# adityamwagh/SuperSLAM

Hardware: AMD Instinct MI355X
Metric: stereo pairs/sec (SPx2+LG) at 1376x376 (higher is better)
Workload: dtype f16; 1 GPU; configs[1]: SuperPoint x2 + select + gather + 1x LightGlue on 1376x376 stereo pairs; a step = 8 x 64 = 512 pairs per GPU resident in HBM (8 library calls of 64 pairs, different images per call), max_keypoints 600, seeded synthetic weights; pairs_per_call=64, max_keypoints=600, matches_last_call=1412, parallelism=replicated weights, pairs sharded over 1 rank(s), no data-path collective

## Files before the change

superslam_amd/csrc/sp_convs.hip:

```cpp
#include <cstdlib>
#include <string>

#include "igemm.h"
#include "kernels.h"

namespace sship {

static IgemmArgs conv_args(const ConvW& w, const _Float16* in, int B, int H, int W) {
  IgemmArgs a{};
  a.in0 = in; a.in1 = in; a.cin0 = w.cin; a.cs0 = w.cin; a.cs1 = w.cin;
  a.wpack = w.w; a.bias = w.bias; a.B = B; a.H = H; a.W = W; a.cout = w.cout; a.ostride = w.cout;
  return a;
}

hipError_t sp_conv1x1_f16(const ConvW& w, const _Float16* in, _Float16* out, int B, int H, int W, hipStream_t s) {
  IgemmArgs a = conv_args(w, in, B, H, W);
  a.out0 = out;
  if (w.cin != 256) return hipErrorInvalidValue;
  return launch_igemm<1, 256, 128, 4, EpiF16<false, false>>(a, w.cout_pad, s);
}

typedef float f4x_t __attribute__((ext_vector_type(4)));
__global__ __launch_bounds__(256, 2) void k_convpb_stream(const _Float16* __restrict__ in, const _Float16* __restrict__ w,
                                                          const float* __restrict__ bias, float* __restrict__ out, int P,
                                                          int ostride) {
  __shared__ __attribute__((aligned(16))) _Float16 s_a4[8 * 512];
  const int lane = threadIdx.x & 63, n = lane & 15, kb = lane >> 4;
  for (int u = threadIdx.x; u < 8 * 64; u += 256) {
    const int ks = u >> 6, l = u & 63;
    *reinterpret_cast<uint4*>(s_a4 + u * 8) = *reinterpret_cast<const uint4*>(w + (size_t)(64 + (l & 15)) * 256 + ks * 32 + (l >> 4) * 8);
  }
  h8_t a[4][8];
#pragma unroll
  for (int m = 0; m < 4; ++m)
#pragma unroll
    for (int ks = 0; ks < 8; ++ks) a[m][ks] = *reinterpret_cast<const h8_t*>(w + (size_t)(16 * m + n) * 256 + ks * 32 + kb * 8);
  __shared__ __attribute__((aligned(16))) float s_b[80];
  if (threadIdx.x < 80) s_b[threadIdx.x] = threadIdx.x < 65 ? bias[threadIdx.x] : 0.f;
  __syncthreads();
  const int ntiles = (P + 15) >> 4, nwaves = gridDim.x * 4;
  const _Float16* src = in + kb * 8;
  h8_t fA[8], fB[8];
  auto fetch = [&](h8_t (&f)[8], int t) __attribute__((always_inline)) {
    const int pix = min(min(t, ntiles - 1) * 16 + n, P - 1);
    const _Float16* p = src + (size_t)pix * 256;
#pragma unroll
    for (int ks = 0; ks < 8; ++ks) f[ks] = *reinterpret_cast<const h8_t*>(p + ks * 32);
  };
  auto tile = [&](const h8_t (&f)[8], int t) __attribute__((always_inline)) {
    f4x_t acc[5];
#pragma unroll
    for (int m = 0; m < 5; ++m) acc[m] = *reinterpret_cast<const f4x_t*>(s_b + 16 * m + 4 * kb);
#pragma unroll
    for (int ks = 0; ks < 8; ++ks) {
      const h8_t a4 = *reinterpret_cast<const h8_t*>(s_a4 + (ks * 64 + lane) * 8);
#pragma unroll
      for (int m = 0; m < 4; ++m) acc[m] = __builtin_amdgcn_mfma_f32_16x16x32_f16(a[m][ks], f[ks], acc[m], 0, 0, 0);
      acc[4] = __builtin_amdgcn_mfma_f32_16x16x32_f16(a4, f[ks], acc[4], 0, 0, 0);
    }
    const int pix = t * 16 + n;
    if (pix < P) {
      float* o = out + (size_t)pix * ostride + 4 * kb;
#pragma unroll
      for (int m = 0; m < 4; ++m) *reinterpret_cast<f4x_t*>(o + 16 * m) = acc[m];
      if (kb == 0) o[64] = acc[4][0];
    }
  };
  const int t0 = blockIdx.x * 4 + (threadIdx.x >> 6);
  fetch(fA, t0);
  for (int t = t0; t < ntiles; t += 2 * nwaves) {
    fetch(fB, t + nwaves);
    __builtin_amdgcn_sched_barrier(0);
    tile(fA, t);
    if (t + nwaves < ntiles) {
      fetch(fA, t + 2 * nwaves);
      __builtin_amdgcn_sched_barrier(0);
      tile(fB, t + nwaves);
    }
  }
}

hipError_t sp_conv1x1_f32(const ConvW& w, const _Float16* in, float* out, int ostride, int B, int H, int W,
                          hipStream_t s) {
  if (w.cin != 256) return hipErrorInvalidValue;
  static const bool use_igemm = dev_env("SUPERSLAM_HIP_CONVPB") && std::string(dev_env("SUPERSLAM_HIP_CONVPB")) == "igemm";
  if (w.w_q && w.cout == 65 && ostride >= 68 && ostride % 4 == 0 && !use_igemm) {
    const int P = B * H * W;
    int wgs = 2 * cu_count();
    if (wgs * 4 > (P + 15) / 16) wgs = ((P + 15) / 16 + 3) / 4;
    hipLaunchKernelGGL(k_convpb_stream, dim3(wgs), dim3(256), 0, s, in, w.w_q, w.bias, out, P, ostride);
    return hipGetLastError();
  }
#if SSHIP_DEV_SWITCHES
  IgemmArgs a = conv_args(w, in, B, H, W);
  a.out0 = out; a.ostride = ostride;
  return launch_igemm<1, 256, 96, 4, EpiF32>(a, w.cout_pad, s);
#else
  return hipErrorInvalidValue;
#endif
}

constexpr int kDhLd = 264;
__global__ __launch_bounds__(512) void k_desc_head_gather(const _Float16* __restrict__ da, int Hc, int Wc,
                                                          const int* __restrict__ cell_h, const int* __restrict__ cell_w,
                                                          const int* __restrict__ n_dev, int max_kp,
                                                          const _Float16* __restrict__ wp, const float* __restrict__ bias,
                                                          _Float16* __restrict__ out, size_t out_img_stride) {
  __shared__ __attribute__((aligned(16))) _Float16 s_x[64 * kDhLd];
  __shared__ float s_red[8][64];
  const int b = blockIdx.y, i0 = blockIdx.x * 64;
  const int n = n_dev[b];
  if (i0 >= n) return;
  const int tid = threadIdx.x, wave = tid >> 6, lane = tid & 63, j = lane & 31, hh = lane >> 5;
  const _Float16* img = da + (size_t)b * Hc * Wc * 256;
  for (int u = tid; u < 64 * 32; u += 512) {
    const int r = u >> 5, part = u & 31;
    uint4 v = make_uint4(0, 0, 0, 0);
    if (i0 + r < n) {
      const int ch = cell_h[(size_t)b * max_kp + i0 + r], cw = cell_w[(size_t)b * max_kp + i0 + r];
      v = *reinterpret_cast<const uint4*>(img + ((size_t)ch * Wc + cw) * 256 + part * 8);
    }
    *reinterpret_cast<uint4*>(s_x + r * kDhLd + part * 8) = v;
  }
  h8_t a[16];
  {
    const _Float16* w = wp + (size_t)wave * (16 * 512) + lane * 8;
#pragma unroll
    for (int ks = 0; ks < 16; ++ks) a[ks] = *reinterpret_cast<const h8_t*>(w + ks * 512);
  }
  __syncthreads();
  f16x_t acc[2];
#pragma unroll
  for (int nn = 0; nn < 2; ++nn)
#pragma unroll
    for (int r = 0; r < 16; ++r) acc[nn][r] = 0.f;
#pragma unroll
  for (int ks = 0; ks < 16; ++ks) {
    const h8_t b0 = *reinterpret_cast<const h8_t*>(s_x + j * kDhLd + ks * 16 + hh * 8);
    const h8_t b1 = *reinterpret_cast<const h8_t*>(s_x + (32 + j) * kDhLd + ks * 16 + hh * 8);
    acc[0] = mfma32(a[ks], b0, acc[0]);
    acc[1] = mfma32(a[ks], b1, acc[1]);
  }
  float v[2][16];
#pragma unroll
  for (int g = 0; g < 4; ++g) {
    const float4 bv = *reinterpret_cast<const float4*>(bias + wave * 32 + hh * 4 + g * 8);
    const float bb[4] = {bv.x, bv.y, bv.z, bv.w};
#pragma unroll
    for (int nn = 0; nn < 2; ++nn)
#pragma unroll
      for (int e = 0; e < 4; ++e) v[nn][4 * g + e] = (float)(_Float16)(acc[nn][4 * g + e] + bb[e]);
  }
  auto row_sum_sq = [&](float (&tot)[2]) {
#pragma unroll
    for (int nn = 0; nn < 2; ++nn) {
      float ss = 0.f;
#pragma unroll
      for (int r = 0; r < 16; ++r) ss += v[nn][r] * v[nn][r];
      ss += __shfl_xor(ss, 32, 64);
      if (hh == 0) s_red[wave][nn * 32 + j] = ss;
    }
    __syncthreads();
#pragma unroll
    for (int nn = 0; nn < 2; ++nn) {
      float t = 0.f;
#pragma unroll
      for (int w = 0; w < 8; ++w) t += s_red[w][nn * 32 + j];
      tot[nn] = t;
    }
    __syncthreads();
  };
  float tot[2];
  row_sum_sq(tot);
#pragma unroll
  for (int nn = 0; nn < 2; ++nn) {
    const float denom = fmaxf(sqrtf(tot[nn]), 1e-12f);
#pragma unroll
    for (int r = 0; r < 16; ++r) v[nn][r] = (float)(_Float16)(v[nn][r] / denom);
  }
  row_sum_sq(tot);
#pragma unroll
  for (int nn = 0; nn < 2; ++nn) {
    const int i = i0 + nn * 32 + j;
    if (i >= n) continue;
    const float inv = rsqrtf(tot[nn] + 1e-12f);
    _Float16* orow = out + (size_t)b * out_img_stride + (size_t)i * 256 + wave * 32 + hh * 4;
#pragma unroll
    for (int g = 0; g < 4; ++g)
      *reinterpret_cast<h4_t*>(orow + g * 8) =
          to_h4(v[nn][4 * g] * inv, v[nn][4 * g + 1] * inv, v[nn][4 * g + 2] * inv, v[nn][4 * g + 3] * inv);
  }
}

constexpr int kDsPatchLd = 584;
template <int NN, bool BIL = false>
__global__ __launch_bounds__(512) void k_desc_head_sparse(const _Float16* __restrict__ a4b, int Hc, int Wc,
                                                          const int* __restrict__ cell_h, const int* __restrict__ cell_w,
                                                          const int* __restrict__ n_dev, int max_kp,
                                                          const _Float16* __restrict__ wda, const float* __restrict__ bda,
                                                          const _Float16* __restrict__ wdb, const float* __restrict__ bdb,
                                                          _Float16* __restrict__ out, size_t out_img_stride) {
  extern __shared__ __attribute__((aligned(16))) char ds_smem[];
  _Float16* s_p = reinterpret_cast<_Float16*>(ds_smem);
  constexpr int NK = 32 * NN;
  _Float16* s_x = s_p + NK * kDsPatchLd;
  float (*s_red)[64] = reinterpret_cast<float (*)[64]>(s_x + NK * kDhLd);
  int* s_cell = reinterpret_cast<int*>(s_red + 8);
  float* s_wt = reinterpret_cast<float*>(s_cell + 64);
  const int b = blockIdx.y, i0 = blockIdx.x * (BIL ? NK / 4 : NK);
  const int n = min(max(n_dev[b], 0), max_kp);
  if (i0 >= n) return;
  const int tid = threadIdx.x, wave = tid >> 6, lane = tid & 63, j = lane & 31, hh = lane >> 5;
  if constexpr (BIL) {
    if (tid < NK) {
      const int i = i0 + (tid >> 2), q = tid & 3;
      int c = -1;
      float wq = 0.f;
      if (i < n) {
        const int px = cell_h[(size_t)b * max_kp + i];
        int x0, y0;
        float fx, fy;
        bilinear_corner((float)(px & 0xffff), (float)(px >> 16), Hc, Wc, x0, y0, fx, fy);
        const int cy = y0 + (q >> 1), cx = x0 + (q & 1);
        if (cy >= 0 && cy < Hc && cx >= 0 && cx < Wc) { c = (cy << 16) | cx; wq = bilinear_weight(q, fx, fy); }
      }
      s_cell[tid] = c;
      s_wt[tid] = wq;
    }
  } else {
    if (tid < NK)
      s_cell[tid] = i0 + tid < n ? (cell_h[(size_t)b * max_kp + i0 + tid] << 16) | cell_w[(size_t)b * max_kp + i0 + tid] : -1;
  }
  const _Float16* img = a4b + (size_t)b * Hc * Wc * 128;
  f16x_t acc[NN];
#pragma unroll
  for (int g = 0; g < 4; ++g) {
    const float4 bv = *reinterpret_cast<const float4*>(bda + wave * 32 + hh * 4 + g * 8);
#pragma unroll
    for (int nn = 0; nn < NN; ++nn) { acc[nn][4 * g] = bv.x; acc[nn][4 * g + 1] = bv.y; acc[nn][4 * g + 2] = bv.z; acc[nn][4 * g + 3] = bv.w; }
  }
  const _Float16* wa = wda + (size_t)wave * (72 * 512) + lane * 8;
  auto frag_of = [](int idx, int& tap, int& ks) __attribute__((always_inline)) {
    const int h32 = idx / 18, r18 = idx - 18 * h32, t6 = r18 / 3, ky = r18 - 3 * t6;
    tap = ky * 3 + (t6 >> 1); ks = 2 * h32 + (t6 & 1);
  };
  auto wfrag = [&](int lin) __attribute__((always_inline)) {
    int tap, ks;
    frag_of(lin % 36, tap, ks);
    return *reinterpret_cast<const h8_t*>(wa + (((lin / 36) * 9 + tap) * 4 + ks) * 512);
  };
  h8_t fa[2][12];
#pragma unroll
  for (int i = 0; i < 12; ++i) fa[0][i] = wfrag(i);
  __syncthreads();
#pragma unroll
  for (int chunk = 0; chunk < 2; ++chunk) {
    if (chunk) __syncthreads();
    for (int u = tid; u < NK * 72; u += 512) {
      const int kp = u / 72, rem = u - kp * 72, tap = rem >> 3, part = rem & 7;
      const int ky = tap / 3, kx = tap - ky * 3;
      const int c = s_cell[kp];
      const int y = (c >> 16) + ky - 1, x = (c & 0xffff) + kx - 1;
      uint4 v = make_uint4(0, 0, 0, 0);
      if (c >= 0 && y >= 0 && y < Hc && x >= 0 && x < Wc)
        v = *reinterpret_cast<const uint4*>(img + ((size_t)y * Wc + x) * 128 + chunk * 64 + part * 8);
      *reinterpret_cast<uint4*>(s_p + kp * kDsPatchLd + tap * 64 + part * 8) = v;
    }
    __syncthreads();
#pragma unroll
    for (int grp = 0; grp < 3; ++grp) {
      const int g_lin = chunk * 3 + grp;
      if (g_lin + 1 < 6) {
#pragma unroll
        for (int i = 0; i < 12; ++i) fa[(g_lin + 1) & 1][i] = wfrag((g_lin + 1) * 12 + i);
      }
      __builtin_amdgcn_sched_barrier(0);
#pragma unroll
      for (int i = 0; i < 12; ++i) {
        int tap, ks;
        frag_of(grp * 12 + i, tap, ks);
#pragma unroll
        for (int nn = 0; nn < NN; ++nn) {
          const h8_t bf = *reinterpret_cast<const h8_t*>(s_p + (nn * 32 + j) * kDsPatchLd + tap * 64 + ks * 16 + hh * 8);
          acc[nn] = mfma32(fa[g_lin & 1][i], bf, acc[nn]);
        }
      }
    }
  }
  h8_t a[16];
  {
    const _Float16* w = wdb + (size_t)wave * (16 * 512) + lane * 8;
#pragma unroll
    for (int ks = 0; ks < 16; ++ks) a[ks] = *reinterpret_cast<const h8_t*>(w + ks * 512);
  }
#pragma unroll
  for (int g = 0; g < 4; ++g) {
#pragma unroll
    for (int nn = 0; nn < NN; ++nn)
      *reinterpret_cast<h4_t*>(s_x + (nn * 32 + j) * kDhLd + wave * 32 + hh * 4 + g * 8) =
          to_h4(fmaxf(acc[nn][4 * g], 0.f), fmaxf(acc[nn][4 * g + 1], 0.f), fmaxf(acc[nn][4 * g + 2], 0.f), fmaxf(acc[nn][4 * g + 3], 0.f));
  }
  __syncthreads();
#pragma unroll
  for (int nn = 0; nn < NN; ++nn)
#pragma unroll
    for (int r = 0; r < 16; ++r) acc[nn][r] = 0.f;
#pragma unroll
  for (int ks = 0; ks < 16; ++ks) {
#pragma unroll
    for (int nn = 0; nn < NN; ++nn) {
      const h8_t bf = *reinterpret_cast<const h8_t*>(s_x + (nn * 32 + j) * kDhLd + ks * 16 + hh * 8);
      acc[nn] = mfma32(a[ks], bf, acc[nn]);
    }
  }
  float v[NN][16];
#pragma unroll
  for (int g = 0; g < 4; ++g) {
    const float4 bv = *reinterpret_cast<const float4*>(bdb + wave * 32 + hh * 4 + g * 8);
    const float bb[4] = {bv.x, bv.y, bv.z, bv.w};
#pragma unroll
    for (int nn = 0; nn < NN; ++nn)
#pragma unroll
      for (int e = 0; e < 4; ++e) v[nn][4 * g + e] = (float)(_Float16)(acc[nn][4 * g + e] + bb[e]);
  }
  auto row_sum_sq = [&](float (&tot)[NN]) {
#pragma unroll
    for (int nn = 0; nn < NN; ++nn) {
      float ss = 0.f;
#pragma unroll
      for (int r = 0; r < 16; ++r) ss += v[nn][r] * v[nn][r];
      ss += __shfl_xor(ss, 32, 64);
      if (hh == 0) s_red[wave][nn * 32 + j] = ss;
    }
    __syncthreads();
#pragma unroll
    for (int nn = 0; nn < NN; ++nn) {
      float t = 0.f;
#pragma unroll
      for (int w = 0; w < 8; ++w) t += s_red[w][nn * 32 + j];
      tot[nn] = t;
    }
    __syncthreads();
  };
  float tot[NN];
  row_sum_sq(tot);
#pragma unroll
  for (int nn = 0; nn < NN; ++nn) {
    const float denom = fmaxf(sqrtf(tot[nn]), 1e-12f);
#pragma unroll
    for (int r = 0; r < 16; ++r) v[nn][r] = (float)(_Float16)(v[nn][r] / denom);
  }
  if constexpr (BIL) {
#pragma unroll
    for (int nn = 0; nn < NN; ++nn) {
      const float wq = s_wt[nn * 32 + j];
#pragma unroll
      for (int r = 0; r < 16; ++r) {
        float t = v[nn][r] * wq;
        t += __shfl_xor(t, 1, 64);
        t += __shfl_xor(t, 2, 64);
        v[nn][r] = t;
      }
    }
    row_sum_sq(tot);
#pragma unroll
    for (int nn = 0; nn < NN; ++nn) {
      const int i = i0 + ((nn * 32 + j) >> 2), q = j & 3;
      if (i >= n) continue;
      const float denom = fmaxf(sqrtf(tot[nn]), 1e-12f);
      _Float16* orow = out + (size_t)b * out_img_stride + (size_t)i * 256 + wave * 32 + hh * 4;
#pragma unroll
      for (int g = 0; g < 4; ++g)
        if (q == g)
          *reinterpret_cast<h4_t*>(orow + g * 8) =
              to_h4(v[nn][4 * g] / denom, v[nn][4 * g + 1] / denom, v[nn][4 * g + 2] / denom, v[nn][4 * g + 3] / denom);
    }
    return;
  }
  row_sum_sq(tot);
#pragma unroll
  for (int nn = 0; nn < NN; ++nn) {
    const int i = i0 + nn * 32 + j;
    if (i >= n) continue;
    const float inv = rsqrtf(tot[nn] + 1e-12f);
    _Float16* orow = out + (size_t)b * out_img_stride + (size_t)i * 256 + wave * 32 + hh * 4;
#pragma unroll
    for (int g = 0; g < 4; ++g)
      *reinterpret_cast<h4_t*>(orow + g * 8) =
          to_h4(v[nn][4 * g] * inv, v[nn][4 * g + 1] * inv, v[nn][4 * g + 2] * inv, v[nn][4 * g + 3] * inv);
  }
}

hipError_t launch_desc_head_sparse_bilinear(const ConvW& da32, const ConvW& db32, const _Float16* a4b, int Hc, int Wc, const int* pix,
                                            const int* n_dev, int max_kp, int B, _Float16* out, size_t out_img_stride, hipStream_t s) {
  if (da32.cin != 128 || da32.cout != 256 || da32.ct != 32 || da32.ks != 3) return hipErrorInvalidValue;
  if (Hc > 4095 || Wc > 8191) return hipErrorInvalidValue;
  constexpr size_t smem = (size_t)64 * kDsPatchLd * 2 + (size_t)64 * kDhLd * 2 + 8 * 64 * 4 + 64 * 4 + 64 * 4;
  static const hipError_t attr_rc = [] {
    hipError_t e = hipFuncSetAttribute(reinterpret_cast<const void*>(k_desc_head_sparse<2, true>), hipFuncAttributeMaxDynamicSharedMemorySize, (int)smem);
    if (e != hipSuccess) return e;
    return hipFuncSetAttribute(reinterpret_cast<const void*>(k_desc_head_sparse<1, true>), hipFuncAttributeMaxDynamicSharedMemorySize, (int)smem);
  }();
  if (attr_rc != hipSuccess) return attr_rc;
  if (B * ((max_kp + 15) / 16) * 2 <= cu_count())
    hipLaunchKernelGGL((k_desc_head_sparse<1, true>), dim3((max_kp + 7) / 8, B), dim3(512), smem, s, a4b, Hc, Wc, pix, nullptr, n_dev,
                       max_kp, da32.w, da32.bias, db32.w, db32.bias, out, out_img_stride);
  else
    hipLaunchKernelGGL((k_desc_head_sparse<2, true>), dim3((max_kp + 15) / 16, B), dim3(512), smem, s, a4b, Hc, Wc, pix, nullptr, n_dev,
                       max_kp, da32.w, da32.bias, db32.w, db32.bias, out, out_img_stride);
  return hipGetLastError();
}

hipError_t launch_desc_head_sparse(const ConvW& da32, const ConvW& db32, const _Float16* a4b, int Hc, int Wc, const int* cell_h,
                                   const int* cell_w, const int* n_dev, int max_kp, int B, _Float16* out, size_t out_img_stride,
                                   hipStream_t s) {
  if (da32.cin != 128 || da32.cout != 256 || da32.ct != 32 || da32.ks != 3) return hipErrorInvalidValue;
  constexpr size_t smem = (size_t)64 * kDsPatchLd * 2 + (size_t)64 * kDhLd * 2 + 8 * 64 * 4 + 64 * 4;
  static const hipError_t attr_rc = [] {
    hipError_t e = hipFuncSetAttribute(reinterpret_cast<const void*>(k_desc_head_sparse<2>), hipFuncAttributeMaxDynamicSharedMemorySize, (int)smem);
    if (e != hipSuccess) return e;
    return hipFuncSetAttribute(reinterpret_cast<const void*>(k_desc_head_sparse<1>), hipFuncAttributeMaxDynamicSharedMemorySize, (int)smem);
  }();
  if (attr_rc != hipSuccess) return attr_rc;
  if (B * ((max_kp + 63) / 64) * 2 <= cu_count())
    hipLaunchKernelGGL(k_desc_head_sparse<1>, dim3((max_kp + 31) / 32, B), dim3(512), smem, s, a4b, Hc, Wc, cell_h, cell_w, n_dev,
                       max_kp, da32.w, da32.bias, db32.w, db32.bias, out, out_img_stride);
  else
    hipLaunchKernelGGL(k_desc_head_sparse<2>, dim3((max_kp + 63) / 64, B), dim3(512), smem, s, a4b, Hc, Wc, cell_h, cell_w, n_dev,
                       max_kp, da32.w, da32.bias, db32.w, db32.bias, out, out_img_stride);
  return hipGetLastError();
}

void launch_desc_head_gather(const ConvW& db32, const _Float16* da, int Hc, int Wc, const int* cell_h, const int* cell_w,
                             const int* n_dev, int max_kp, int B, _Float16* out, size_t out_img_stride, hipStream_t s) {
  hipLaunchKernelGGL(k_desc_head_gather, dim3((max_kp + 63) / 64, B), dim3(512), 0, s, da, Hc, Wc, cell_h, cell_w, n_dev,
                     max_kp, db32.w, db32.bias, out, out_img_stride);
}

}
```

Before: 5613 pairs/s.

## Add double-buffered direct-to-LDS staged sparse descriptor head kernel

Adds a new sparse descriptor-head kernel that stages the 3x3 patch per keypoint in four channel halves. Each half is loaded into two ping-pong LDS buffers with global_load_lds_dwordx4 and an XOR swizzle, so the next half loads while MFMAs run on the current one. The LDS footprint drops and the convDa tile reuses a patch buffer, which lets 4 blocks fit per CU. The throughput (non-latency) path now defaults to this kernel, the old kernel stays reachable through dev switches, and the shared tail is factored into a device function. The inline asm that manipulates m0 and the swizzled indexing add correctness risk.

```diff
diff --git a/superslam_amd/csrc/sp_convs.hip b/superslam_amd/csrc/sp_convs.hip
--- a/superslam_amd/csrc/sp_convs.hip
+++ b/superslam_amd/csrc/sp_convs.hip
@@ -185,6 +185,115 @@
     if (i >= n) continue;
     const float inv = rsqrtf(tot[nn] + 1e-12f);
     _Float16* orow = out + (size_t)b * out_img_stride + (size_t)i * 256 + wave * 32 + hh * 4;
+#pragma unroll
+    for (int g = 0; g < 4; ++g)
+      *reinterpret_cast<h4_t*>(orow + g * 8) =
+          to_h4(v[nn][4 * g] * inv, v[nn][4 * g + 1] * inv, v[nn][4 * g + 2] * inv, v[nn][4 * g + 3] * inv);
+  }
+}
+
+template <int NN, bool BIL>
+__device__ __forceinline__ void desc_head_tail(f16x_t (&acc)[NN], _Float16* s_x, float (*s_red)[64], const float* s_wt,
+                                               const _Float16* __restrict__ wdb, const float* __restrict__ bdb,
+                                               _Float16* __restrict__ out, int i0, int n) {
+  const int tid = threadIdx.x, wave = tid >> 6, lane = tid & 63, j = lane & 31, hh = lane >> 5;
+  h8_t a[16];
+  {
+    const _Float16* w = wdb + (size_t)wave * (16 * 512) + lane * 8;
+#pragma unroll
+    for (int ks = 0; ks < 16; ++ks) a[ks] = *reinterpret_cast<const h8_t*>(w + ks * 512);
+  }
+#pragma unroll
+  for (int g = 0; g < 4; ++g) {
+#pragma unroll
+    for (int nn = 0; nn < NN; ++nn)
+      *reinterpret_cast<h4_t*>(s_x + (nn * 32 + j) * kDhLd + wave * 32 + hh * 4 + g * 8) =
+          to_h4(fmaxf(acc[nn][4 * g], 0.f), fmaxf(acc[nn][4 * g + 1], 0.f), fmaxf(acc[nn][4 * g + 2], 0.f), fmaxf(acc[nn][4 * g + 3], 0.f));
+  }
+  __syncthreads();
+#pragma unroll
+  for (int nn = 0; nn < NN; ++nn)
+#pragma unroll
+    for (int r = 0; r < 16; ++r) acc[nn][r] = 0.f;
+#pragma unroll
+  for (int ks = 0; ks < 16; ++ks) {
+#pragma unroll
+    for (int nn = 0; nn < NN; ++nn) {
+      const h8_t bf = *reinterpret_cast<const h8_t*>(s_x + (nn * 32 + j) * kDhLd + ks * 16 + hh * 8);
+      acc[nn] = mfma32(a[ks], bf, acc[nn]);
+    }
+  }
+  float v[NN][16];
+#pragma unroll
+  for (int g = 0; g < 4; ++g) {
+    const float4 bv = *reinterpret_cast<const float4*>(bdb + wave * 32 + hh * 4 + g * 8);
+    const float bb[4] = {bv.x, bv.y, bv.z, bv.w};
+#pragma unroll
+    for (int nn = 0; nn < NN; ++nn)
+#pragma unroll
+      for (int e = 0; e < 4; ++e) v[nn][4 * g + e] = (float)(_Float16)(acc[nn][4 * g + e] + bb[e]);
+  }
+  auto row_sum_sq = [&](float (&tot)[NN]) {
+#pragma unroll
+    for (int nn = 0; nn < NN; ++nn) {
+      float ss = 0.f;
+#pragma unroll
+      for (int r = 0; r < 16; ++r) ss += v[nn][r] * v[nn][r];
+      ss += __shfl_xor(ss, 32, 64);
+      if (hh == 0) s_red[wave][nn * 32 + j] = ss;
+    }
+    __syncthreads();
+#pragma unroll
+    for (int nn = 0; nn < NN; ++nn) {
+      float t = 0.f;
+#pragma unroll
+      for (int w = 0; w < 8; ++w) t += s_red[w][nn * 32 + j];
+      tot[nn] = t;
+    }
+    __syncthreads();
+  };
+  float tot[NN];
+  row_sum_sq(tot);
+#pragma unroll
+  for (int nn = 0; nn < NN; ++nn) {
+    const float denom = fmaxf(sqrtf(tot[nn]), 1e-12f);
+#pragma unroll
+    for (int r = 0; r < 16; ++r) v[nn][r] = (float)(_Float16)(v[nn][r] / denom);
+  }
+  if constexpr (BIL) {
+#pragma unroll
+    for (int nn = 0; nn < NN; ++nn) {
+      const float wq = s_wt[nn * 32 + j];
+#pragma unroll
+      for (int r = 0; r < 16; ++r) {
+        float t = v[nn][r] * wq;
+        t += __shfl_xor(t, 1, 64);
+        t += __shfl_xor(t, 2, 64);
+        v[nn][r] = t;
+      }
+    }
+    row_sum_sq(tot);
+#pragma unroll
+    for (int nn = 0; nn < NN; ++nn) {
+      const int i = i0 + ((nn * 32 + j) >> 2), q = j & 3;
+      if (i >= n) continue;
+      const float denom = fmaxf(sqrtf(tot[nn]), 1e-12f);
+      _Float16* orow = out + (size_t)i * 256 + wave * 32 + hh * 4;
+#pragma unroll
+      for (int g = 0; g < 4; ++g)
+        if (q == g)
+          *reinterpret_cast<h4_t*>(orow + g * 8) =
+              to_h4(v[nn][4 * g] / denom, v[nn][4 * g + 1] / denom, v[nn][4 * g + 2] / denom, v[nn][4 * g + 3] / denom);
+    }
+    return;
+  }
+  row_sum_sq(tot);
+#pragma unroll
+  for (int nn = 0; nn < NN; ++nn) {
+    const int i = i0 + nn * 32 + j;
+    if (i >= n) continue;
+    const float inv = rsqrtf(tot[nn] + 1e-12f);
+    _Float16* orow = out + (size_t)i * 256 + wave * 32 + hh * 4;
 #pragma unroll
     for (int g = 0; g < 4; ++g)
       *reinterpret_cast<h4_t*>(orow + g * 8) =
@@ -287,126 +396,166 @@
       }
     }
   }
-  h8_t a[16];
-  {
-    const _Float16* w = wdb + (size_t)wave * (16 * 512) + lane * 8;
-#pragma unroll
-    for (int ks = 0; ks < 16; ++ks) a[ks] = *reinterpret_cast<const h8_t*>(w + ks * 512);
-  }
+  desc_head_tail<NN, BIL>(acc, s_x, s_red, s_wt, wdb, bdb, out + (size_t)b * out_img_stride, i0, n);
+}
+
+constexpr int kDuRows = 64;
+constexpr int kDuHalfBytes = 9 * kDuRows * 64;
+constexpr int kDuG = 6, kDuD = 2;
+__device__ __attribute__((aligned(16))) const unsigned g_du_zero[4] = {0u, 0u, 0u, 0u};
+template <bool BIL>
+__global__ __launch_bounds__(512, 4) void k_desc_head_sparse_units(const _Float16* __restrict__ a4b, int Hc, int Wc,
+                                                                   const int* __restrict__ cell_h, const int* __restrict__ cell_w,
+                                                                   const int* __restrict__ n_dev, int max_kp,
+                                                                   const _Float16* __restrict__ wda, const float* __restrict__ bda,
+                                                                   const _Float16* __restrict__ wdb, const float* __restrict__ bdb,
+                                                                   _Float16* __restrict__ out, size_t out_img_stride) {
+  extern __shared__ __attribute__((aligned(16))) char ds_smem[];
+  char* s_buf = ds_smem;
+  _Float16* s_x = reinterpret_cast<_Float16*>(ds_smem);
+  float (*s_red)[64] = reinterpret_cast<float (*)[64]>(ds_smem + 2 * kDuHalfBytes);
+  int* s_cell = reinterpret_cast<int*>(s_red + 8);
+  float* s_wt = reinterpret_cast<float*>(s_cell + 64);
+  static_assert(kDuRows * kDhLd * 2 <= kDuHalfBytes, "the convDa tile fits in one patch buffer");
+  const int b = blockIdx.y, i0 = blockIdx.x * (BIL ? kDuRows / 4 : kDuRows);
+  const int n = min(max(n_dev[b], 0), max_kp);
+  if (i0 >= n) return;
+  const int tid = threadIdx.x, wave = tid >> 6, lane = tid & 63, j = lane & 31, hh = lane >> 5;
+  if (tid < kDuRows) {
+    int c = -1;
+    if constexpr (BIL) {
+      const int i = i0 + (tid >> 2), q = tid & 3;
+      float wq = 0.f;
+      if (i < n) {
+        const int px = cell_h[(size_t)b * max_kp + i];
+        int x0, y0;
+        float fx, fy;
+        bilinear_corner((float)(px & 0xffff), (float)(px >> 16), Hc, Wc, x0, y0, fx, fy);
+        const int cy = y0 + (q >> 1), cx = x0 + (q & 1);
+        if (cy >= 0 && cy < Hc && cx >= 0 && cx < Wc) { c = (cy << 16) | cx; wq = bilinear_weight(q, fx, fy); }
+      }
+      s_wt[tid] = wq;
+    } else {
+      if (i0 + tid < n) c = (cell_h[(size_t)b * max_kp + i0 + tid] << 16) | cell_w[(size_t)b * max_kp + i0 + tid];
+    }
+    s_cell[tid] = c;
+  }
+  const _Float16* img = a4b + (size_t)b * Hc * Wc * 128;
+  f16x_t acc[2];
 #pragma unroll
   for (int g = 0; g < 4; ++g) {
-#pragma unroll
-    for (int nn = 0; nn < NN; ++nn)
-      *reinterpret_cast<h4_t*>(s_x + (nn * 32 + j) * kDhLd + wave * 32 + hh * 4 + g * 8) =
-          to_h4(fmaxf(acc[nn][4 * g], 0.f), fmaxf(acc[nn][4 * g + 1], 0.f), fmaxf(acc[nn][4 * g + 2], 0.f), fmaxf(acc[nn][4 * g + 3], 0.f));
-  }
+    const float4 bv = *reinterpret_cast<const float4*>(bda + wave * 32 + hh * 4 + g * 8);
+#pragma unroll
+    for (int nn = 0; nn < 2; ++nn) { acc[nn][4 * g] = bv.x; acc[nn][4 * g + 1] = bv.y; acc[nn][4 * g + 2] = bv.z; acc[nn][4 * g + 3] = bv.w; }
+  }
+  const _Float16* wa = wda + (size_t)wave * (72 * 512) + lane * 8;
+  auto frag_of = [](int lin, int& chunk, int& tap, int& ks2) __attribute__((always_inline)) {
+    chunk = lin / 36;
+    const int r18 = lin % 18, t6 = r18 / 3, ky = r18 - 3 * t6;
+    tap = ky * 3 + (t6 >> 1); ks2 = t6 & 1;
+  };
+  auto wfrag = [&](int lin) __attribute__((always_inline)) {
+    int chunk, tap, ks2;
+    frag_of(lin, chunk, tap, ks2);
+    return *reinterpret_cast<const h8_t*>(wa + ((chunk * 9 + tap) * 4 + 2 * ((lin / 18) & 1) + ks2) * 512);
+  };
+  h8_t fa[kDuD][kDuG];
+#pragma unroll
+  for (int g = 0; g < kDuD - 1; ++g)
+#pragma unroll
+    for (int i = 0; i < kDuG; ++i) fa[g][i] = wfrag(g * kDuG + i);
   __syncthreads();
-#pragma unroll
-  for (int nn = 0; nn < NN; ++nn)
-#pragma unroll
-    for (int r = 0; r < 16; ++r) acc[nn][r] = 0.f;
-#pragma unroll
-  for (int ks = 0; ks < 16; ++ks) {
-#pragma unroll
-    for (int nn = 0; nn < NN; ++nn) {
-      const h8_t bf = *reinterpret_cast<const h8_t*>(s_x + (nn * 32 + j) * kDhLd + ks * 16 + hh * 8);
-      acc[nn] = mfma32(a[ks], bf, acc[nn]);
-    }
-  }
-  float v[NN][16];
-#pragma unroll
-  for (int g = 0; g < 4; ++g) {
-    const float4 bv = *reinterpret_cast<const float4*>(bdb + wave * 32 + hh * 4 + g * 8);
-    const float bb[4] = {bv.x, bv.y, bv.z, bv.w};
-#pragma unroll
-    for (int nn = 0; nn < NN; ++nn)
-#pragma unroll
-      for (int e = 0; e < 4; ++e) v[nn][4 * g + e] = (float)(_Float16)(acc[nn][4 * g + e] + bb[e]);
-  }
-  auto row_sum_sq = [&](float (&tot)[NN]) {
-#pragma unroll
-    for (int nn = 0; nn < NN; ++nn) {
-      float ss = 0.f;
-#pragma unroll
-      for (int r = 0; r < 16; ++r) ss += v[nn][r] * v[nn][r];
-      ss += __shfl_xor(ss, 32, 64);
-      if (hh == 0) s_red[wave][nn * 32 + j] = ss;
-    }
-    __syncthreads();
-#pragma unroll
-    for (int nn = 0; nn < NN; ++nn) {
-      float t = 0.f;
-#pragma unroll
-      for (int w = 0; w < 8; ++w) t += s_red[w][nn * 32 + j];
-      tot[nn] = t;
-    }
-    __syncthreads();
-  };
-  float tot[NN];
-  row_sum_sq(tot);
-#pragma unroll
-  for (int nn = 0; nn < NN; ++nn) {
-    const float denom = fmaxf(sqrtf(tot[nn]), 1e-12f);
-#pragma unroll
-    for (int r = 0; r < 16; ++r) v[nn][r] = (float)(_Float16)(v[nn][r] / denom);
-  }
-  if constexpr (BIL) {
-#pragma unroll
-    for (int nn = 0; nn < NN; ++nn) {
-      const float wq = s_wt[nn * 32 + j];
-#pragma unroll
-      for (int r = 0; r < 16; ++r) {
-        float t = v[nn][r] * wq;
-        t += __shfl_xor(t, 1, 64);
-        t += __shfl_xor(t, 2, 64);
-        v[nn][r] = t;
-      }
-    }
-    row_sum_sq(tot);
-#pragma unroll
-    for (int nn = 0; nn < NN; ++nn) {
-      const int i = i0 + ((nn * 32 + j) >> 2), q = j & 3;
-      if (i >= n) continue;
-      const float denom = fmaxf(sqrtf(tot[nn]), 1e-12f);
-      _Float16* orow = out + (size_t)b * out_img_stride + (size_t)i * 256 + wave * 32 + hh * 4;
-#pragma unroll
-      for (int g = 0; g < 4; ++g)
-        if (q == g)
-          *reinterpret_cast<h4_t*>(orow + g * 8) =
-              to_h4(v[nn][4 * g] / denom, v[nn][4 * g + 1] / denom, v[nn][4 * g + 2] / denom, v[nn][4 * g + 3] / denom);
-    }
-    return;
-  }
-  row_sum_sq(tot);
-#pragma unroll
-  for (int nn = 0; nn < NN; ++nn) {
-    const int i = i0 + nn * 32 + j;
-    if (i >= n) continue;
-    const float inv = rsqrtf(tot[nn] + 1e-12f);
-    _Float16* orow = out + (size_t)b * out_img_stride + (size_t)i * 256 + wave * 32 + hh * 4;
-#pragma unroll
-    for (int g = 0; g < 4; ++g)
-      *reinterpret_cast<h4_t*>(orow + g * 8) =
-          to_h4(v[nn][4 * g] * inv, v[nn][4 * g + 1] * inv, v[nn][4 * g + 2] * inv, v[nn][4 * g + 3] * inv);
-  }
+  const int wave_s = __builtin_amdgcn_readfirstlane(wave);
+  const int cell = s_cell[(wave_s & 3) * 16 + (lane >> 2)];
+  auto stage_half = [&](int half) __attribute__((always_inline)) {
+    const unsigned dst0 = (unsigned)(uintptr_t)(s_buf + (half & 1) * kDuHalfBytes);
+    int c = cell;
+    asm volatile("" : "+v"(c));
+    const int cy = c >> 16, cx = c & 0xffff;
+    const int part = (lane & 3) ^ ((lane >> 4) & 3);
+    const _Float16* src0 = img + ((ptrdiff_t)cy * Wc + cx) * 128 + half * 32 + part * 8;
+#pragma unroll
+    for (int k = 0; k < 5; ++k) {
+      const int p = wave_s + 8 * k;
+      if (p < 36) {
+        const int tap = p >> 2, ky = tap / 3, kx = tap - 3 * ky;
+        const int y = cy + ky - 1, x = cx + kx - 1;
+        const bool ok = c >= 0 && y >= 0 && y < Hc && x >= 0 && x < Wc;
+        const void* gsrc = ok ? static_cast<const void*>(src0 + ((ptrdiff_t)(ky - 1) * Wc + (kx - 1)) * 128)
+                              : static_cast<const void*>(g_du_zero);
+        const unsigned lds_dst = __builtin_amdgcn_readfirstlane(dst0 + (unsigned)p * 1024u);
+        unsigned keep;
+        asm volatile("s_mov_b32 %0, m0\n\ts_mov_b32 m0, %2\n\ts_nop 0\n\tglobal_load_lds_dwordx4 %1, off\n\ts_mov_b32 m0, %0"
+                     : "=&s"(keep) : "v"(gsrc), "s"(lds_dst) : "memory");
+      }
+    }
+  };
+  stage_half(0);
+#pragma unroll
+  for (int half = 0; half < 4; ++half) {
+    asm volatile("s_waitcnt vmcnt(0) lgkmcnt(0)\n\ts_barrier" ::: "memory");
+    const char* s_p = s_buf + (half & 1) * kDuHalfBytes;
+#pragma unroll
+    for (int grp = 0; grp < 3; ++grp) {
+      const int g_lin = half * 3 + grp;
+      if (g_lin + kDuD - 1 < 12) {
+#pragma unroll
+        for (int i = 0; i < kDuG; ++i) fa[(g_lin + kDuD - 1) % kDuD][i] = wfrag((g_lin + kDuD - 1) * kDuG + i);
+      }
+      __builtin_amdgcn_sched_barrier(0);
+      if (grp == 0 && half + 1 < 4) stage_half(half + 1);
+#pragma unroll
+      for (int i = 0; i < kDuG; ++i) {
+        int chunk, tap, ks2;
+        frag_of(g_lin * kDuG + i, chunk, tap, ks2);
+#pragma unroll
+        for (int nn = 0; nn < 2; ++nn) {
+          const h8_t bf = *reinterpret_cast<const h8_t*>(s_p + (tap * kDuRows + nn * 32 + j) * 64 + (((ks2 * 2 + hh) ^ (j >> 2)) & 3) * 16);
+          acc[nn] = mfma32(fa[g_lin % kDuD][i], bf, acc[nn]);
+        }
+      }
+    }
+  }
+  desc_head_tail<2, BIL>(acc, s_x, s_red, s_wt, wdb, bdb, out + (size_t)b * out_img_stride, i0, n);
+}
+
+constexpr size_t kDuSmem = 2 * (size_t)kDuHalfBytes + 8 * 64 * 4 + 64 * 4 + 64 * 4;
+constexpr size_t kDsSmem = (size_t)64 * kDsPatchLd * 2 + (size_t)64 * kDhLd * 2 + 8 * 64 * 4 + 64 * 4 + 64 * 4;
+static int desc_head_form(bool latency) {
+#if SSHIP_DEV_SWITCHES
+  static const std::string mode = [] { const char* e = dev_env("SUPERSLAM_HIP_DESC"); return std::string(e ? e : ""); }();
+  if (mode == "serial_all") return 2;
+  if (mode == "units_all") return 1;
+  if (mode == "serial" && !latency) return 2;
+#endif
+  return latency ? 0 : 1;
 }
 
 hipError_t launch_desc_head_sparse_bilinear(const ConvW& da32, const ConvW& db32, const _Float16* a4b, int Hc, int Wc, const int* pix,
                                             const int* n_dev, int max_kp, int B, _Float16* out, size_t out_img_stride, hipStream_t s) {
   if (da32.cin != 128 || da32.cout != 256 || da32.ct != 32 || da32.ks != 3) return hipErrorInvalidValue;
   if (Hc > 4095 || Wc > 8191) return hipErrorInvalidValue;
-  constexpr size_t smem = (size_t)64 * kDsPatchLd * 2 + (size_t)64 * kDhLd * 2 + 8 * 64 * 4 + 64 * 4 + 64 * 4;
+  constexpr size_t smem = kDsSmem;
   static const hipError_t attr_rc = [] {
-    hipError_t e = hipFuncSetAttribute(reinterpret_cast<const void*>(k_desc_head_sparse<2, true>), hipFuncAttributeMaxDynamicSharedMemorySize, (int)smem);
+    hipError_t e = hipFuncSetAttribute(reinterpret_cast<const void*>(k_desc_head_sparse_units<true>), hipFuncAttributeMaxDynamicSharedMemorySize, (int)kDuSmem);
+#if SSHIP_DEV_SWITCHES
+    if (e == hipSuccess) e = hipFuncSetAttribute(reinterpret_cast<const void*>(k_desc_head_sparse<2, true>), hipFuncAttributeMaxDynamicSharedMemorySize, (int)smem);
+#endif
     if (e != hipSuccess) return e;
     return hipFuncSetAttribute(reinterpret_cast<const void*>(k_desc_head_sparse<1, true>), hipFuncAttributeMaxDynamicSharedMemorySize, (int)smem);
   }();
   if (attr_rc != hipSuccess) return attr_rc;
-  if (B * ((max_kp + 15) / 16) * 2 <= cu_count())
+  const int form = desc_head_form(B * ((max_kp + 15) / 16) * 2 <= cu_count());
+  if (form == 0)
     hipLaunchKernelGGL((k_desc_head_sparse<1, true>), dim3((max_kp + 7) / 8, B), dim3(512), smem, s, a4b, Hc, Wc, pix, nullptr, n_dev,
                        max_kp, da32.w, da32.bias, db32.w, db32.bias, out, out_img_stride);
+#if SSHIP_DEV_SWITCHES
+  else if (form == 2)
+    hipLaunchKernelGGL((k_desc_head_sparse<2, true>), dim3((max_kp + 15) / 16, B), dim3(512), smem, s, a4b, Hc, Wc, pix, nullptr, n_dev,
+                       max_kp, da32.w, da32.bias, db32.w, db32.bias, out, out_img_stride);
+#endif
   else
-    hipLaunchKernelGGL((k_desc_head_sparse<2, true>), dim3((max_kp + 15) / 16, B), dim3(512), smem, s, a4b, Hc, Wc, pix, nullptr, n_dev,
+    hipLaunchKernelGGL(k_desc_head_sparse_units<true>, dim3((max_kp + 15) / 16, B), dim3(512), kDuSmem, s, a4b, Hc, Wc, pix, nullptr, n_dev,
                        max_kp, da32.w, da32.bias, db32.w, db32.bias, out, out_img_stride);
   return hipGetLastError();
 }
@@ -415,18 +564,27 @@
                                    const int* cell_w, const int* n_dev, int max_kp, int B, _Float16* out, size_t out_img_stride,
                                    hipStream_t s) {
   if (da32.cin != 128 || da32.cout != 256 || da32.ct != 32 || da32.ks != 3) return hipErrorInvalidValue;
-  constexpr size_t smem = (size_t)64 * kDsPatchLd * 2 + (size_t)64 * kDhLd * 2 + 8 * 64 * 4 + 64 * 4;
+  constexpr size_t smem = kDsSmem - 64 * 4;
   static const hipError_t attr_rc = [] {
-    hipError_t e = hipFuncSetAttribute(reinterpret_cast<const void*>(k_desc_head_sparse<2>), hipFuncAttributeMaxDynamicSharedMemorySize, (int)smem);
+    hipError_t e = hipFuncSetAttribute(reinterpret_cast<const void*>(k_desc_head_sparse_units<false>), hipFuncAttributeMaxDynamicSharedMemorySize, (int)kDuSmem);
+#if SSHIP_DEV_SWITCHES
+    if (e == hipSuccess) e = hipFuncSetAttribute(reinterpret_cast<const void*>(k_desc_head_sparse<2>), hipFuncAttributeMaxDynamicSharedMemorySize, (int)smem);
+#endif
     if (e != hipSuccess) return e;
     return hipFuncSetAttribute(reinterpret_cast<const void*>(k_desc_head_sparse<1>), hipFuncAttributeMaxDynamicSharedMemorySize, (int)smem);
   }();
   if (attr_rc != hipSuccess) return attr_rc;
-  if (B * ((max_kp + 63) / 64) * 2 <= cu_count())
+  const int form = desc_head_form(B * ((max_kp + 63) / 64) * 2 <= cu_count());
+  if (form == 0)
     hipLaunchKernelGGL(k_desc_head_sparse<1>, dim3((max_kp + 31) / 32, B), dim3(512), smem, s, a4b, Hc, Wc, cell_h, cell_w, n_dev,
                        max_kp, da32.w, da32.bias, db32.w, db32.bias, out, out_img_stride);
+#if SSHIP_DEV_SWITCHES
+  else if (form == 2)
+    hipLaunchKernelGGL(k_desc_head_sparse<2>, dim3((max_kp + 63) / 64, B), dim3(512), smem, s, a4b, Hc, Wc, cell_h, cell_w, n_dev,
+                       max_kp, da32.w, da32.bias, db32.w, db32.bias, out, out_img_stride);
+#endif
   else
-    hipLaunchKernelGGL(k_desc_head_sparse<2>, dim3((max_kp + 63) / 64, B), dim3(512), smem, s, a4b, Hc, Wc, cell_h, cell_w, n_dev,
+    hipLaunchKernelGGL(k_desc_head_sparse_units<false>, dim3((max_kp + kDuRows - 1) / kDuRows, B), dim3(512), kDuSmem, s, a4b, Hc, Wc, cell_h, cell_w, n_dev,
                        max_kp, da32.w, da32.bias, db32.w, db32.bias, out, out_img_stride);
   return hipGetLastError();
 }
```

After: 5647 pairs/s, median of 6. No clear change (+0.6%).
